# magenta/music-spectrogram-diffusion

Measured on AMD Instinct MI355X. Metric: mel-frames/sec, higher is better.
Workload: dtype f16x3 (operands split into hi + lo half planes, 3 f16 MFMAs per product, fp32 accumulate; fp32 residual/norm/softmax/sampler); 1 GPU; base_with_context, 1000-step DDPM, CFG w=5, 1 song(s) per GPU, segment-sequential with context hand-off, 5 segments of 256 frames per GPU; precision=f16x3, precision_requested=f16x3, parallelism=song-parallel x1, mode=replicas, attention_query_planes=library default: hi + lo for Q and for the softmax weights, knobs=library defaults

## Files before the change

### music-spectrogram-diffusion_amd/build_native.py

```python
from __future__ import annotations

import os
import shutil
import subprocess
import sys

HERE = os.path.dirname(os.path.abspath(__file__))
ROOT = os.path.dirname(HERE)
CSRC = os.path.join(HERE, 'csrc')
EXP = os.path.join(ROOT, 'tools', 'ubench', 'exp')
LIB = os.path.join(CSRC, 'libmsd_amd.so')
LIB_EXP = os.path.join(EXP, 'libmsd_amd_exp.so')
LIBS = {'f16': (LIB, []), 'bf16': (os.path.join(CSRC, 'libmsd_amd_bf16.so'), ['-DMSD_PLANE_BF16=1'])}
EXP_SRC = os.path.join(EXP, 'src_r04')
EXP_LIBS = {'exp': (LIB_EXP, ['-DMSD_EXPERIMENTS=1'])}
SOURCES = ['msd_api.hip']
HEADERS = ['common.h', 'phase_stamps.h', 'gemm_h16.h', 'gemm_f32.h', 'attention.h', 'elementwise.h',
           os.path.join('..', '..', 'include', 'msd_amd.h')]
EXP_HEADERS = ['chain.h', 'gemm_h16_exp.h', 'gemm_splitk_exchange.inc', 'gemm_h16_pair.h', 'gemm_h16_wide.h', 'gemm_h16_ls.h']


def _hipcc():
  for c in (os.environ.get('HIPCC'), shutil.which('hipcc'), '/opt/rocm/bin/hipcc'):
    if c and os.path.exists(c):
      return c
  raise RuntimeError('hipcc not found (ROCm toolchain required to build the HIP library)')


def needs_build(lib: str = LIB) -> bool:
  if not os.path.exists(lib):
    return True
  t = os.path.getmtime(lib)
  if os.path.abspath(lib) == os.path.abspath(LIB_EXP):
    deps = [os.path.join(EXP_SRC, f) for f in os.listdir(EXP_SRC)] + [os.path.join(EXP, f) for f in EXP_HEADERS]
  else:
    deps = [os.path.join(CSRC, f) for f in SOURCES + HEADERS + [os.path.join('..', 'build_native.py')]]
  return any(os.path.getmtime(f) > t for f in deps)


def check_prefetch_registers(listing: str) -> str:
  tool = os.path.join(HERE, 'check_prefetch_regs.py')
  if not os.path.exists(tool):
    raise RuntimeError('%s is missing: the build cannot verify the prefetch registers of the library' % tool)
  out = subprocess.run([sys.executable, tool, listing], capture_output=True, text=True)
  if out.returncode != 0:
    raise RuntimeError('prefetch register check failed on %s:\n%s\n%s' % (listing, out.stdout[-3000:], out.stderr[-2000:]))
  return out.stdout.strip().split('\n')[-1]


NO_SCRATCH_KERNELS = ('sampler_step_kernel', 'threefry_normal_kernel')


def check_no_scratch(listing: str, kernels=NO_SCRATCH_KERNELS) -> str:
  import re
  text = open(listing).read()
  seen = {k: 0 for k in kernels}
  bad = []
  for m in re.finditer(r'^\s*\.amdhsa_kernel\s+(\S+)(.*?)^\s*\.end_amdhsa_kernel', text, flags=re.M | re.S):
    name, body = m.group(1), m.group(2)
    for k in kernels:
      if k in name:
        seen[k] += 1
        size = re.search(r'\.amdhsa_private_segment_fixed_size\s+(\d+)', body)
        dyn = re.search(r'\.amdhsa_uses_dynamic_stack\s+(\d+)', body)
        if size is None or int(size.group(1)) != 0 or (dyn is not None and int(dyn.group(1)) != 0):
          bad.append('%s: private segment %s, dynamic stack %s' % (name, size.group(1) if size else '?', dyn.group(1) if dyn else '0'))
  missing = [k for k, c in seen.items() if c == 0]
  if missing:
    raise RuntimeError('scratch check: no kernel descriptor of %s in %s' % (missing, listing))
  if bad:
    raise RuntimeError('scratch check failed on %s: these kernels use scratch memory:\n  %s' % (listing, '\n  '.join(bad)))
  return 'OK: no scratch in ' + ', '.join('%d x %s' % (c, k) for k, c in seen.items())


def build(force: bool = False, verbose: bool = True, experiments: bool = False) -> str:
  import tempfile
  targets = [(lib, defs, CSRC) for lib, defs in LIBS.values()]
  if experiments:
    if not os.path.isdir(EXP_SRC):
      raise RuntimeError('%s is missing: run `bash tools/ubench/exp/restore_src_r04.sh` first (the experiments build needs round 4\'s sources)' % EXP_SRC)
    targets += [(lib, defs, EXP_SRC) for lib, defs in EXP_LIBS.values()]
  for lib, defs, src in targets:
    if not force and not needs_build(lib):
      continue
    with tempfile.TemporaryDirectory(prefix='msd_build_') as tmp:
      out = os.path.join(tmp, os.path.basename(lib))
      cmd = [_hipcc(), '--offload-arch=gfx950', '-O3', '-std=c++17', '-fPIC', '-shared', '-save-temps',
             '-fno-gpu-rdc', '-Wno-unused-result', '-ffile-prefix-map=%s=.' % ROOT, '-ffile-prefix-map=%s=.' % tmp,
             '-cuid=msd_amd',
             '-I', src] + defs + ['-o', os.path.basename(lib)] + [os.path.join(src, s) for s in SOURCES]
      if verbose:
        print('[build_native]', ' '.join(cmd), flush=True)
      subprocess.run(cmd, check=True, cwd=tmp)
      listings = [os.path.join(tmp, f) for f in os.listdir(tmp) if f.endswith('.s') and 'gfx950' in f]
      if not listings:
        raise RuntimeError('no gfx950 device listing (*gfx950*.s, -save-temps) in %s: cannot verify the prefetch '
                           'registers; the scratch directory holds %s' % (tmp, sorted(os.listdir(tmp))))
      for l in listings:
        verdict = check_prefetch_registers(l)
        if verbose:
          print('[build_native] prefetch registers:', verdict, flush=True)
        if src == CSRC:
          verdict = check_no_scratch(l)
          if verbose:
            print('[build_native] scratch:', verdict, flush=True)
      shutil.copyfile(out, lib + '.tmp')
      os.chmod(lib + '.tmp', 0o755)
      os.replace(lib + '.tmp', lib)
  return LIB


if __name__ == '__main__':
  build(force='--force' in sys.argv, experiments='--experiments' in sys.argv)
  print(LIB)
```

### music-spectrogram-diffusion_amd/csrc/gemm_h16.h

```cpp
#pragma once
#include <type_traits>
#include "common.h"
#include "phase_stamps.h"

namespace msd {

struct PrefetchTarget {
  const char* base[2] = {nullptr, nullptr};
  int rows = 0;
  int row_stride = 0;
  int lpr = 0;
  int lg = 0;
  void set(const void* p0, const void* p1, int rows_, int row_stride_, int row_bytes) {
    base[0] = static_cast<const char*>(p0); base[1] = static_cast<const char*>(p1);
    rows = rows_; row_stride = row_stride_; lpr = (row_bytes + 127) >> 7;
    lg = 0;
    while ((1 << lg) < lpr) ++lg;
  }
};
constexpr int kMaxPrefetchTargets = 1;
struct WeightPrefetch {
  PrefetchTarget t[kMaxPrefetchTargets];
  int n = 0;
  void add(const PrefetchTarget& x) { if (x.rows > 0 && n < kMaxPrefetchTargets) t[n++] = x; }
};

constexpr int kPrefetchPerThread = 3;
template <int PF>
struct PrefetchRegsT { uint32_t r[PF > 0 ? PF * kPrefetchPerThread : 1]; };
enum { kPfNone = 0 };
__host__ __device__ inline int prefetch_kind(const WeightPrefetch& pf) { return pf.n; }

template <int PF>
__device__ __forceinline__ void prefetch_weights(const WeightPrefetch& pf, int blk, int nblk, const void* valid,
                                                 PrefetchRegsT<PF>& keep) {
  if constexpr (PF == kPfNone) {
    keep.r[0] = 0;
    return;
  } else {
    const int wave = __builtin_amdgcn_readfirstlane((int)threadIdx.x >> 6), nwave = (int)blockDim.x >> 6;
    const int lane = (int)threadIdx.x & 63;
#pragma unroll
    for (int k = 0; k < PF; ++k) {
      const PrefetchTarget& t = pf.t[k];
      const int rows = t.rows, lpr = t.lpr;
      const int planes = t.base[1] && t.base[1] != t.base[0] ? 2 : 1;
      const int rpt = 64 >> t.lg;
      const int sub = lane >> t.lg, line = lane & ((1 << t.lg) - 1);
      const uint32_t lane_off = (uint32_t)sub * (uint32_t)t.row_stride + (uint32_t)line * 128u;
#pragma unroll
      for (int u = 0; u < kPrefetchPerThread; ++u) {
        const int rp0 = ((blk + nblk * u) * nwave + wave) * rpt;
        const int pl = (planes == 2 && rp0 >= rows) ? 1 : 0, row0 = rp0 - pl * rows;
        const char* row_ptr = t.base[pl] + (size_t)row0 * t.row_stride;
        const bool in = rp0 < rows * planes && row0 + sub < rows && line < lpr;
        const char* src = in ? row_ptr + lane_off : reinterpret_cast<const char*>(valid);
        asm volatile("global_load_dword %0, %1, off ; msd_prefetch" : "=&v"(keep.r[k * kPrefetchPerThread + u]) : "v"(src) : "memory");
      }
    }
  }
}
template <int PF>
__device__ __forceinline__ void prefetch_done(const PrefetchRegsT<PF>& keep) {
#pragma unroll
  for (int u = 0; u < (PF > 0 ? PF * kPrefetchPerThread : 1); ++u) asm volatile("" ::"v"(keep.r[u]));
}

constexpr bool kPfWave = true;
constexpr bool kPfWaveAttn = true;
template <int PF, bool LDS_SINK = false>
__device__ __forceinline__ void prefetch_wave(const WeightPrefetch& pf, int blk, int nblk, const void* valid,
                                              char* sink_lds = nullptr) {
  if constexpr (PF != kPfNone) {
    constexpr int TOUCHES = 4 * kPrefetchPerThread;
    const int lane = (int)threadIdx.x & 63;
    uint32_t sink = 0;
#pragma unroll
    for (int k = 0; k < PF; ++k) {
      const PrefetchTarget& t = pf.t[k];
      const int rows = t.rows, lpr = t.lpr;
      const int planes = t.base[1] && t.base[1] != t.base[0] ? 2 : 1;
      const int rpt = 64 >> t.lg;
      const int sub = lane >> t.lg, line = lane & ((1 << t.lg) - 1);
      const uint32_t lane_off = (uint32_t)sub * (uint32_t)t.row_stride + (uint32_t)line * 128u;
#pragma unroll
      for (int u = 0; u < TOUCHES; ++u) {
        const int rp0 = (blk + nblk * u) * rpt;
        const int pl = (planes == 2 && rp0 >= rows) ? 1 : 0, row0 = rp0 - pl * rows;
        const char* row_ptr = t.base[pl] + (size_t)row0 * t.row_stride;
        const bool in = rp0 < rows * planes && row0 + sub < rows && line < lpr;
        const char* src = in ? row_ptr + lane_off : reinterpret_cast<const char*>(valid);
        if constexpr (LDS_SINK) {
          typedef const __attribute__((address_space(1))) void* pf_gptr_t;
          typedef __attribute__((address_space(3))) void* pf_lptr_t;
          __builtin_amdgcn_global_load_lds((pf_gptr_t)src, (pf_lptr_t)(size_t)(unsigned)(size_t)sink_lds, 4, 0, 0);
        } else {
          asm volatile("global_load_dword %0, %1, off ; msd_prefetch" : "+v"(sink) : "v"(src) : "memory");
        }
      }
    }
    asm volatile("" ::"v"(sink));
  }
}

struct GemmParams {
  const h16_t* A[2];
  const h16_t* B[2];
  int lda, ldb;
  int M, N, K;
  WeightPrefetch pf;
  int pf_nblk = 0;
  int xcd_rows = 1;
  int xcd_walk_n = 0;
  struct TileMap {
    int nbm = 0, nbn = 0;
    int nbm_x = 1, nbn_x = 1;
    int cx_log2 = 3;
    unsigned inv_nbm_x = 0, inv_nbn_x = 0;
    void fill(int M, int N, int BM, int BN, int rx) {
      const int cx = 8 / rx;
      nbm = M / BM; nbn = N / BN;
      nbm_x = (nbm + rx - 1) / rx; nbn_x = (nbn + cx - 1) / cx;
      cx_log2 = cx == 8 ? 3 : (cx == 4 ? 2 : (cx == 2 ? 1 : 0));
      inv_nbm_x = nbm_x > 1 ? (unsigned)((0x100000000ull + (unsigned)nbm_x - 1) / (unsigned)nbm_x) : 0u;
      inv_nbn_x = nbn_x > 1 ? (unsigned)((0x100000000ull + (unsigned)nbn_x - 1) / (unsigned)nbn_x) : 0u;
    }
  } map;
  unsigned* sat = nullptr;
  unsigned sat_tag = 1;
};

struct SatFlag {
  unsigned* p = nullptr;
  unsigned tag = 1;
};

typedef __attribute__((ext_vector_type(8))) plane_elem mfma_h16x8;
typedef __attribute__((ext_vector_type(4))) unsigned int u32x4;

__device__ __forceinline__ mfma_h16x8 as_frag(uint4 v) {
  union { uint4 u; mfma_h16x8 f; } c;
  c.u = v;
  return c.f;
}

__device__ __forceinline__ mfma_h16x8 ld_frag16(const h16_t* p) {
  return as_frag(*reinterpret_cast<const uint4*>(p));
}

__device__ __forceinline__ int vt_perm16(int o) { return 8 * ((o >> 2) & 1) + (o & 3) + 4 * (o >> 3); }

constexpr int kSlabPad = 4;
constexpr int kGemmBK = 64;

__device__ __forceinline__ int lds_tile_off(int row, int chunk) {
  return row * 128 + ((chunk ^ (row & 7)) << 4);
}

template <int BM, int BN>
struct GemmAcc {
  static constexpr int FM = BM / 32, FN = BN / 32;
  f32x4 a[FM][FN];
};

template <int NP, int BM, int BN, int NS, class Epi, int PF = kPfNone, bool PROLOGUE = true, bool REG_EPI = false>
__device__ __forceinline__ void gemm_tile(const GemmParams& p, const Epi& epi, int bm, int bn, char* smem,
                                          GemmAcc<BM, BN>* acc_out = nullptr, int ts_blk = -1, bool fresh = false) {
#if MSD_TIMESTAMPS
  const int msd_ts_blk = ts_blk >= 0 ? ts_blk : (int)blockIdx.x;
#endif
  constexpr bool W13 = BN == 48;
  static_assert(!W13 || (NP == 2 && BM == 32), "1 x 3 wave layout: 32 x 48 tiles, two planes");
  constexpr int WM = W13 ? BM : BM / 2, WN = W13 ? 16 : BN / 2;
  constexpr int FM = WM / 16, FN = WN / 16;
  constexpr int A_BYTES = BM * 128, B_BYTES = BN * 128;
  constexpr int STAGE_BYTES = NP * (A_BYTES + B_BYTES);
  constexpr int A_LD = BM / 32, B_LD = BN / 32;
  constexpr int B_Q = W13 ? BN / 16 : NP * B_LD;
  constexpr int PW = NP * A_LD + B_Q;
  constexpr int LDS_LD = BN + kSlabPad;
  static_assert((BM * LDS_LD + BM) * 4 <= NS * STAGE_BYTES, "epilogue slab must fit the operand LDS");

  const int tid = threadIdx.x, lane = tid & 63;
  const int wave = __builtin_amdgcn_readfirstlane(tid >> 6);
  const int wm = W13 ? 0 : wave >> 1, wn = W13 ? (wave < 2 ? wave : 2) : wave & 1;
  const int m0 = bm * BM, n0 = bn * BN;

  const int r8 = lane >> 3, csrc = (lane & 7) ^ r8;
  const h16_t* ga[NP];
  const h16_t* gb[NP];
#pragma unroll
  for (int pl = 0; pl < NP; ++pl) {
    ga[pl] = p.A[pl] + (size_t)(m0 + wave * (BM / 4) + r8) * p.lda + csrc * 8;
    gb[pl] = W13 ? p.B[wave >> 1] + (size_t)(n0 + (wave & 1) * (BN / 2) + r8) * p.ldb + csrc * 8
                 : p.B[pl] + (size_t)(n0 + wave * (BN / 4) + r8) * p.ldb + csrc * 8;
  }
  const size_t a_step = (size_t)8 * p.lda, b_step = (size_t)8 * p.ldb;
#define MSD_A_SRC(PL, I, K0) (ga[PL] + (I) * a_step + (K0))
  typedef const __attribute__((address_space(1))) void* gptr_t;
  typedef __attribute__((address_space(3))) void* lptr_t;

#define MSD_D_ISSUE1(KT, BUF, Q)                                                             \
  {                                                                                          \
    char* base_ = smem + (BUF) * STAGE_BYTES;                                                \
    const int k0_ = (KT) * kGemmBK;                                                          \
    if constexpr (W13) {                                                                     \
      if ((Q) < NP * A_LD)                                                                   \
        __builtin_amdgcn_global_load_lds((gptr_t)(MSD_A_SRC((Q) / A_LD, (Q) % A_LD, k0_)),   \
            (lptr_t)(base_ + ((Q) / A_LD) * A_BYTES + (wave * (BM / 4) + 8 * ((Q) % A_LD)) * 128), 16, 0, 0); \
      else                                                                                   \
        __builtin_amdgcn_global_load_lds((gptr_t)(gb[0] + ((Q) - NP * A_LD) * b_step + k0_), \
            (lptr_t)(base_ + NP * A_BYTES + (wave >> 1) * B_BYTES +                          \
                     ((wave & 1) * (BN / 2) + 8 * ((Q) - NP * A_LD)) * 128), 16, 0, 0);      \
    } else {                                                                                 \
      constexpr int AB_ = A_LD + (B_LD ? B_LD : 1);                                          \
      const int     pl_ = (Q) / AB_, r_ = (Q) % AB_;                                         \
      if (r_ < A_LD)                                                                         \
        __builtin_amdgcn_global_load_lds((gptr_t)(MSD_A_SRC(pl_, r_, k0_)),                  \
            (lptr_t)(base_ + pl_ * A_BYTES + (wave * (BM / 4) + 8 * r_) * 128), 16, 0, 0);   \
      else                                                                                   \
        __builtin_amdgcn_global_load_lds((gptr_t)(gb[pl_] + (r_ - A_LD) * b_step + k0_),     \
            (lptr_t)(base_ + NP * A_BYTES + pl_ * B_BYTES + (wave * (BN / 4) + 8 * (r_ - A_LD)) * 128), 16, 0, 0); \
    }                                                                                        \
  }
#define MSD_D_ISSUE(KT, BUF)                                                                \
  { _Pragma("unroll") for (int q0_ = 0; q0_ < PW; ++q0_) MSD_D_ISSUE1(KT, BUF, q0_) }

  f32x4 acc[FM][FN];
#pragma unroll
  for (int i = 0; i < FM; ++i)
#pragma unroll
    for (int j = 0; j < FN; ++j) acc[i][j] = f32x4{0.f, 0.f, 0.f, 0.f};

  const int nk = p.K / kGemmBK;
  MSD_TS_BEGIN((ts_class<BM, BN>()), msd_ts_blk)
  if constexpr (PROLOGUE) {
#pragma unroll
    for (int s = 0; s < NS; ++s)
      if (s < nk) MSD_D_ISSUE(s, s)
  }
  char* const aux = smem + NS * STAGE_BYTES;
  if constexpr (PROLOGUE) epi.template prefetch<BM, BN>(aux, m0, n0, wave, lane);
  __builtin_amdgcn_sched_barrier(0);
  MSD_TS_STAMP(BM, BN, 1)

#define MSD_D_READ(FA, FB, BUF, KK)                                                          \
  {                                                                                          \
    const char* base_ = smem + (BUF) * STAGE_BYTES;                                          \
    const int c_ = (KK) * 4 + (lane >> 4);                                                   \
    _Pragma("unroll") for (int pl = 0; pl < NP; ++pl) {                                      \
      _Pragma("unroll") for (int i = 0; i < FM; ++i)                                         \
        FA[pl][i] = *reinterpret_cast<const mfma_h16x8*>(                                   \
            base_ + pl * A_BYTES + lds_tile_off(wm * WM + i * 16 + (lane & 15), c_));        \
      _Pragma("unroll") for (int j = 0; j < FN; ++j)                                         \
        FB[pl][j] = *reinterpret_cast<const mfma_h16x8*>(                                   \
            base_ + NP * A_BYTES + pl * B_BYTES + lds_tile_off(wn * WN + j * 16 + (lane & 15), c_)); \
    }                                                                                        \
  }

  mfma_h16x8 fa0[NP][FM], fb0[NP][FN], fa1[NP][FM], fb1[NP][FN];
  constexpr int RD = NP * (FM + FN);
  constexpr int MQ = (NP == 2 ? 3 : 1) * FM * FN;
  constexpr int SLOTS = RD > PW ? RD : PW;
  constexpr int MPR = MQ / SLOTS;
  static_assert(W13 || PW == RD, "one DMA and one fragment read per slot");
#define MSD_D_READ1(FA, FB, BUF, KK, Q)                                                      \
  {                                                                                          \
    const int     pl_ = (Q) / (FM + FN), r_ = (Q) % (FM + FN);                               \
    const char* base_ = smem + (BUF) * STAGE_BYTES;                                          \
    const int c_ = (KK) * 4 + (lane >> 4);                                                   \
    if (r_ < FM)                                                                             \
      FA[pl_][r_ < FM ? r_ : 0] = *reinterpret_cast<const mfma_h16x8*>(                     \
          base_ + pl_ * A_BYTES + lds_tile_off(wm * WM + r_ * 16 + (lane & 15), c_));        \
    else                                                                                     \
      FB[pl_][r_ < FM ? 0 : r_ - FM] = *reinterpret_cast<const mfma_h16x8*>(                \
          base_ + NP * A_BYTES + pl_ * B_BYTES + lds_tile_off(wn * WN + (r_ - FM) * 16 + (lane & 15), c_)); \
  }
#define MSD_D_MFMA1(FA, FB, E)                                                               \
  {                                                                                          \
    const int     pr_ = (E) / (FM * FN), t_ = (E) % (FM * FN), i_ = t_ / FN, j_ = t_ % FN;    \
    const int     pb_ = (pr_ == 1) ? NP - 1 : 0, pa_ = (pr_ == 2) ? NP - 1 : 0;              \
    acc[i_][j_] = MSD_MFMA_16X16X32(FB[pb_][j_], FA[pa_][i_], acc[i_][j_], 0, 0, 0); \
  }
#define MSD_D_HALF(DO_ISSUE, KT, BUF_I, FAn, FBn, BUF_R, KK, DO_READ, FAc, FBc)              \
  {                                                                                          \
    _Pragma("unroll") for (int q_ = 0; q_ < SLOTS; ++q_) {                                   \
      if (DO_ISSUE && q_ < PW) MSD_D_ISSUE1(KT, BUF_I, q_)                                   \
      if (DO_READ && q_ < RD) MSD_D_READ1(FAn, FBn, BUF_R, KK, q_)                           \
      _Pragma("unroll") for (int e_ = q_ * MPR; e_ < (q_ + 1 == SLOTS ? MQ : (q_ + 1) * MPR); ++e_) \
        MSD_D_MFMA1(FAc, FBc, e_)                                                            \
      __builtin_amdgcn_sched_barrier(0);                                                     \
    }                                                                                        \
  }
#define MSD_D_BARRIER __builtin_amdgcn_s_barrier();
#define MSD_D_DOISSUE 1
#define MSD_D_STEP(DO_ISSUE, VMWAIT)                                                         \
  {                                                                                          \
    MSD_D_HALF(0, 0, 0, fa1, fb1, buf, 1, 1, fa0, fb0)                                       \
    int nb = buf + 1;                                                                        \
    if (nb == NS) nb = 0;                                                                    \
    asm volatile("s_waitcnt vmcnt(%0)" ::"n"(VMWAIT) : "memory");      \
    __builtin_amdgcn_s_waitcnt(0xC07F);   \
    MSD_D_BARRIER                           \
    __builtin_amdgcn_sched_barrier(0);                                                       \
    MSD_D_HALF(DO_ISSUE, kt + NS, buf, fa0, fb0, nb, 0, 1, fa1, fb1)                         \
     \
     \
     \
    __builtin_amdgcn_s_waitcnt(0xC07F);                                                      \
    buf = nb;                                                                                \
  }

  if ((PROLOGUE || fresh) && nk >= NS) {
    asm volatile("s_waitcnt vmcnt(%0)" ::"n"((NS - 1) * PW) : "memory");
  } else {
    asm volatile("s_waitcnt vmcnt(0)" ::: "memory");
  }
  __builtin_amdgcn_s_barrier();
  __builtin_amdgcn_sched_barrier(0);
  MSD_TS_STAMP(BM, BN, 2)
  MSD_D_READ(fa0, fb0, 0, 0)
  __builtin_amdgcn_s_waitcnt(0xC07F);
  int buf = 0;
  int kt = 0;
  for (; kt + NS < nk; ++kt) MSD_D_STEP(MSD_D_DOISSUE, (NS - 2) * PW)
  if (nk >= NS) {
    if constexpr (NS >= 4) { if (kt + 1 < nk) { MSD_D_STEP(0, (NS - 2) * PW) ++kt; } }
    if constexpr (NS >= 3) { if (kt + 1 < nk) { MSD_D_STEP(0, (NS >= 4 ? NS - 3 : NS - 2) * PW) ++kt; } }
    if constexpr (NS >= 5) { static_assert(NS <= 4, "write the drain ladder for this ring depth"); }
  }
  for (; kt + 1 < nk; ++kt) MSD_D_STEP(0, 0)
  MSD_D_HALF(0, 0, 0, fa1, fb1, buf, 1, 1, fa0, fb0)
  MSD_D_HALF(0, 0, 0, fa0, fb0, buf, 0, 0, fa1, fb1)
#undef MSD_D_STEP
#undef MSD_D_HALF
#undef MSD_D_ISSUE1
#undef MSD_D_READ1
#undef MSD_D_MFMA1
#undef MSD_D_DOISSUE
#undef MSD_D_BARRIER
#undef MSD_D_READ
#undef MSD_D_ISSUE
#undef MSD_A_SRC
  __syncthreads();
  MSD_TS_STAMP(BM, BN, 3)
  if constexpr (REG_EPI) {
    static_assert(!W13, "register epilogues: 2 x 2 wave layout");
#pragma unroll
    for (int i = 0; i < FM; ++i)
#pragma unroll
      for (int j = 0; j < FN; ++j) acc_out->a[i][j] = acc[i][j];
    return;
  } else {
  float* slab = reinterpret_cast<float*>(smem);
  const int lm = lane & 15, ln = (lane >> 4) * 4;
  auto store_slab = [&]() {
    if (W13 && wave == 3) return;
#pragma unroll
    for (int i = 0; i < FM; ++i)
#pragma unroll
      for (int j = 0; j < FN; ++j)
        *reinterpret_cast<float4*>(slab + (size_t)(wm * WM + i * 16 + lm) * LDS_LD + wn * WN + j * 16 + ln) =
            make_float4(acc[i][j][0] * kWScaleInv, acc[i][j][1] * kWScaleInv, acc[i][j][2] * kWScaleInv,
                        acc[i][j][3] * kWScaleInv);
  };
  PrefetchRegsT<PF> pf_keep;
  if constexpr (!kPfWave) prefetch_weights<PF>(p.pf, blockIdx.x, p.pf_nblk > 0 ? p.pf_nblk : (int)gridDim.x, p.B[0], pf_keep);
  else prefetch_weights<kPfNone>(p.pf, 0, 1, nullptr, reinterpret_cast<PrefetchRegsT<kPfNone>&>(pf_keep));
  store_slab();
  epi.template stats<BM, LDS_LD>(slab, m0, tid, aux);
  __syncthreads();
  MSD_TS_STAMP(BM, BN, 4)
  epi.template run<BM, BN, LDS_LD>(slab, m0, n0, tid, aux, true, SatFlag{p.sat, p.sat_tag});
  MSD_TS_STAMP(BM, BN, 5)
  MSD_TS_END((ts_class<BM, BN>()), msd_ts_blk, gridDim.x)
  prefetch_done(pf_keep);
  }
}

__device__ __forceinline__ bool gemm_block_tile(const GemmParams& p, int b, int& bm, int& bn) {
  const GemmParams::TileMap& tm = p.map;
  const int RX = p.xcd_rows, CX = 1 << tm.cx_log2;
  const int xcd = b & 7, tt = b >> 3;
  const int xr = xcd >> tm.cx_log2, xc = xcd & (CX - 1);
  if (p.xcd_walk_n) {
    const int q = tm.nbn_x > 1 ? (int)__umulhi((unsigned)tt, tm.inv_nbn_x) : tt;
    bm = q * RX + xr; bn = (tt - q * tm.nbn_x) * CX + xc;
  } else {
    const int q = tm.nbm_x > 1 ? (int)__umulhi((unsigned)tt, tm.inv_nbm_x) : tt;
    bm = (tt - q * tm.nbm_x) * RX + xr; bn = q * CX + xc;
  }
  return bn < tm.nbn && bm < tm.nbm;
}

constexpr int pf_threads(int pf) { return kPfWave && pf != kPfNone ? 64 : 0; }

template <int NP, int BM, int BN, int NS, class Epi, int PF = kPfNone>
__global__ void __launch_bounds__(256 + pf_threads(PF)) gemm_h16_dma_kernel(GemmParams p, Epi epi) {
  extern __shared__ __attribute__((aligned(16))) char smem[];
  warm_kernargs<kernarg_lines<GemmParams, Epi>()>();
  if constexpr (kPfWave && PF != kPfNone) {
    if (threadIdx.x >= 256) {
      prefetch_wave<PF>(p.pf, blockIdx.x, gridDim.x, p.B[0]);
      return;
    }
  }
  int bm, bn;
  if (!gemm_block_tile(p, (int)blockIdx.x, bm, bn)) return;
  gemm_tile<NP, BM, BN, NS, Epi, PF>(p, epi, bm, bn, smem);
}

template <int LD>
__device__ __forceinline__ void tile_row8(const float* s0, int m, int n, float v[8]) {
  const float4 a0 = *reinterpret_cast<const float4*>(s0 + m * LD + n);
  const float4 a1 = *reinterpret_cast<const float4*>(s0 + m * LD + n + 4);
  v[0] = a0.x; v[1] = a0.y; v[2] = a0.z; v[3] = a0.w;
  v[4] = a1.x; v[5] = a1.y; v[6] = a1.z; v[7] = a1.w;
}

template <int NP>
__device__ __forceinline__ void store_h16x8(h16_t* const* planes, size_t off, const float v[8], RangeCheck& rc) {
  uint32_t wh[4], wl[4];
#pragma unroll
  for (int e = 0; e < 4; ++e) {
    rc.see(v[2 * e], v[2 * e + 1]);
    if (NP == 2) split2_h16(v[2 * e], v[2 * e + 1], wh[e], wl[e]);
    else wh[e] = cvt2_h16(v[2 * e], v[2 * e + 1]);
  }
  *reinterpret_cast<uint4*>(planes[0] + off) = make_uint4(wh[0], wh[1], wh[2], wh[3]);
  if (NP == 2) *reinterpret_cast<uint4*>(planes[1] + off) = make_uint4(wl[0], wl[1], wl[2], wl[3]);
}

struct RowScale {
  const float* ssq = nullptr;
  int tiles = 0;
  float inv_d = 0.f;
  const float* bias = nullptr;
  int bias_step_stride = 0;
  const int* step_ptr = nullptr;
};

constexpr int kAuxMaxTiles = 32;

#ifndef MSD_EPI_AUX_OPTIONAL
#define MSD_EPI_AUX_OPTIONAL 0
#endif
__device__ __forceinline__ bool aux_present(const char* aux) {
#if MSD_EPI_AUX_OPTIONAL
  return aux != nullptr;
#else
  (void)aux;
  return true;
#endif
}

typedef const __attribute__((address_space(1))) void* aux_gptr_t;
typedef __attribute__((address_space(3))) void* aux_lptr_t;

__device__ __forceinline__ aux_lptr_t lds_ptr_of(const void* generic) {
  return (aux_lptr_t)(size_t)(unsigned)(size_t)generic;
}

__device__ __forceinline__ int scan_index(const int* p) {
  int v;
  asm volatile("s_nop 4\n\ts_load_dword %0, %1, 0x0\n\ts_waitcnt lgkmcnt(0)" : "=s"(v) : "s"(p) : "memory");
  return v;
}

__device__ __forceinline__ void aux_dma_linear(const void* g, char* dst, int bytes, int wave, int lane) {
  const int n_instr = (bytes + 1023) >> 10;
  for (int i = wave; i < n_instr; i += 4) {
    int off = i * 1024 + lane * 16;
    off = off < bytes - 16 ? off : bytes - 16;
    __builtin_amdgcn_global_load_lds((aux_gptr_t)((const char*)g + off), lds_ptr_of(dst + i * 1024), 16, 0, 0);
  }
}

__device__ __forceinline__ void aux_dma_row(const void* g, char* dst, int bytes, int lane) {
  int off = lane * 16;
  off = off < bytes - 16 ? off : bytes - 16;
  __builtin_amdgcn_global_load_lds((aux_gptr_t)((const char*)g + off), lds_ptr_of(dst), 16, 0, 0);
}

template <int BM>
constexpr int rowscale_aux_bytes() { return BM * kAuxMaxTiles * 4 + 1024; }
template <int BM>
__host__ __device__ __forceinline__ int rowscale_ssq_bytes(int tiles) { return (BM * tiles * 4 + 1023) & ~1023; }

template <int BM, int BN>
__device__ __forceinline__ void rowscale_prefetch(const RowScale& r, char* aux, int m0, int n0, int wave, int lane) {
  if (!r.ssq) return;
  aux_dma_linear(r.ssq + (size_t)m0 * r.tiles, aux, BM * r.tiles * 4, wave, lane);
  if (r.bias && wave == 3)
    aux_dma_row(r.bias + (size_t)scan_index(r.step_ptr) * r.bias_step_stride + n0, aux + rowscale_ssq_bytes<BM>(r.tiles), BN * 4, lane);
}

typedef const __attribute__((address_space(3))) float* lds_cf32;

typedef const __attribute__((address_space(3))) f32x4* lds_cf32x4;
struct BiasRow {
  lds_cf32 l = nullptr;
  bool present = false;
  __device__ __forceinline__ float at(int i) const { return l[i]; }
  __device__ __forceinline__ void at8(int i, float (&b)[8]) const {
    const f32x4 b0 = reinterpret_cast<lds_cf32x4>(l + i)[0], b1 = reinterpret_cast<lds_cf32x4>(l + i)[1];
    b[0] = b0[0]; b[1] = b0[1]; b[2] = b0[2]; b[3] = b0[3];
    b[4] = b1[0]; b[5] = b1[1]; b[6] = b1[2]; b[7] = b1[3];
  }
};

template <class F>
__device__ __forceinline__ void rowscale_variants(bool folded, bool has_bias, F&& f) {
  if (!folded) f(std::integral_constant<int, 0>{});
  else if (!has_bias) f(std::integral_constant<int, 1>{});
  else f(std::integral_constant<int, 2>{});
}

template <int MODE>
__device__ __forceinline__ void rowscale8(float (&v)[8], float rs, const BiasRow& bias, int i) {
  if constexpr (MODE == 2) {
    float b[8];
    bias.at8(i, b);
#pragma unroll
    for (int e = 0; e < 8; ++e) v[e] = v[e] * rs + b[e];
  } else if constexpr (MODE == 1) {
#pragma unroll
    for (int e = 0; e < 8; ++e) v[e] = v[e] * rs + 0.f;
  }
}

#define MSD_EPI_ITEMS(ITEMS, item)                                             \
  _Pragma("unroll") for (int it_ = 0; it_ < ((ITEMS) + 255) / 256; ++it_)      \
    if (const int item = tid + it_ * 256; ((ITEMS) % 256 == 0) || item < (ITEMS))

template <int BM>
__device__ __forceinline__ void tile_rstd_compute(const RowScale& r, float* rs, int m0, int tid, const char* aux) {
  constexpr int TPR = 256 / BM;
  const int row = tid / TPR, part = tid % TPR;
  float acc = 0.f;
  if (aux_present(aux)) {
    lds_cf32 q = (lds_cf32)(aux) + row * r.tiles;
    constexpr int MAXIT = kAuxMaxTiles / TPR;
    float v[MAXIT];
#pragma unroll
    for (int i = 0; i < MAXIT; ++i) {
      const int t = part + i * TPR;
      v[i] = q[t < r.tiles ? t : part];
    }
#pragma unroll
    for (int i = 0; i < MAXIT; ++i) acc += (part + i * TPR < r.tiles) ? v[i] : 0.f;
  } else {
    const float* q = r.ssq + (size_t)(m0 + row) * r.tiles;
    for (int t = part; t < r.tiles; t += TPR) acc += q[t];
  }
#pragma unroll
  for (int o = 1; o < TPR; o <<= 1) acc += __shfl_xor(acc, o, 64);
  if (part == 0) rs[row] = 1.0f / sqrtf(acc * r.inv_d + 1e-6f);
}

template <int BM>
__device__ __forceinline__ BiasRow tile_rstd(const RowScale& r, float* rs, int m0, int n0, int tid,
                                             const char* aux, bool stats_done = false) {
  if (!stats_done) {
    tile_rstd_compute<BM>(r, rs, m0, tid, aux);
    __syncthreads();
  }
  BiasRow b;
  if (r.bias) {
    if (!aux_present(aux)) __builtin_trap();
    b.present = true;
    b.l = (lds_cf32)(aux + rowscale_ssq_bytes<BM>(r.tiles));
  }
  return b;
}

template <int NP>
struct EpiStoreH16 {
  h16_t* out[2];
  int ldc;
  RowScale rsc;
  template <int BM, int BN> static constexpr int aux_bytes() { return rowscale_aux_bytes<BM>(); }
  template <int BM, int BN>
  __device__ void prefetch(char* aux, int m0, int n0, int wave, int lane) const {
    rowscale_prefetch<BM, BN>(rsc, aux, m0, n0, wave, lane);
  }
  template <int BM, int LD>
  __device__ void stats(float* s0, int m0, int tid, const char* aux) const {
    if (rsc.ssq) tile_rstd_compute<BM>(rsc, s0 + BM * LD, m0, tid, aux);
  }
  template <int BM, int BN, int LD>
  __device__ void run(float* s0, int m0, int n0, int tid, const char* aux = nullptr, bool stats_done = false,
                      SatFlag sf = SatFlag()) const {
    float* rs = s0 + BM * LD;
    BiasRow bias;
    if (rsc.ssq) bias = tile_rstd<BM>(rsc, rs, m0, n0, tid, aux, stats_done);
    RangeCheck rc;
    rowscale_variants(rsc.ssq != nullptr, bias.present, [&](auto mode) {
      MSD_EPI_ITEMS(BM * BN / 8, item) {
        const int m = item / (BN / 8), n = (item % (BN / 8)) * 8;
        float v[8];
        tile_row8<LD>(s0, m, n, v);
        rowscale8<decltype(mode)::value>(v, decltype(mode)::value ? rs[m] : 1.f, bias, n);
        store_h16x8<NP>(out, (size_t)(m0 + m) * ldc + n0 + n, v, rc);
      }
    });
    rc.commit(sf.p, sf.tag);
  }
};

template <int NP>
struct EpiQKV {
  h16_t* qk[2];
  h16_t* vt[2];
  int ld_qk, v_start, seg_len, vt_ld, vt_rows;
  RowScale rsc;
  template <int BM, int BN> static constexpr int aux_bytes() { return rowscale_aux_bytes<BM>(); }
  template <int BM, int BN>
  __device__ void prefetch(char* aux, int m0, int n0, int wave, int lane) const {
    rowscale_prefetch<BM, BN>(rsc, aux, m0, n0, wave, lane);
  }
  template <int BM, int LD>
  __device__ void stats(float* s0, int m0, int tid, const char* aux) const {
    if (rsc.ssq) tile_rstd_compute<BM>(rsc, s0 + BM * LD, m0, tid, aux);
  }
  template <int BM, int BN, int LD>
  __device__ void run(float* s0, int m0, int n0, int tid, const char* aux = nullptr, bool stats_done = false,
                      SatFlag sf = SatFlag()) const {
    float* rs = s0 + BM * LD;
    BiasRow bias;
    if (rsc.ssq) bias = tile_rstd<BM>(rsc, rs, m0, n0, tid, aux, stats_done);
    RangeCheck rc;
    if (n0 < v_start) {
      rowscale_variants(rsc.ssq != nullptr, bias.present, [&](auto mode) {
        MSD_EPI_ITEMS(BM * BN / 8, item) {
          const int m = item / (BN / 8), n = (item % (BN / 8)) * 8;
          float v[8];
// ... 735 lines not shown
```

Measured before the change: 272.0 mel-frames/sec.

## Split LDS-DMA issue across both half steps of the GEMM main loop

```diff
diff --git a/music-spectrogram-diffusion_amd/build_native.py b/music-spectrogram-diffusion_amd/build_native.py
--- a/music-spectrogram-diffusion_amd/build_native.py
+++ b/music-spectrogram-diffusion_amd/build_native.py
@@ -1,6 +1,7 @@
 from __future__ import annotations
 
 import os
+import re
 import shutil
 import subprocess
 import sys
@@ -48,11 +49,162 @@
   return out.stdout.strip().split('\n')[-1]
 
 
+DMA_WAIT_KERNELS = ('gemm_h16_dma_kernel', 'gemm_h16_dual_kernel', 'gemm_h16_geglu_persist_kernel')
+
+
+def _dw_tile_shapes(name):
+  np_ = int(re.search(r'_kernelILi(\d+)E', name).group(1))
+  m = re.search(r'persist_kernelILi\d+ELi(\d+)ELi(\d+)ELi(\d+)E', name)
+  if m:
+    return [(np_,) + tuple(int(x) for x in m.groups())]
+  return [(np_,) + tuple(int(x) for x in t) for t in re.findall(r'Li(\d+)ELi(\d+)ELi(\d+)ENS_', name)]
+
+
+def _dw_dmas_per_wave(np_, bm, bn):
+  return np_ * (bm // 32) + (bn // 16 if bn == 48 else np_ * (bn // 32))
+
+
+def _dw_blocks_of(lines, s, end):
+  out, label, ev, loop = [], 'entry', [], False
+  for j in range(s + 1, end):
+    l = lines[j].split(';')[0].strip()
+    m = re.match(r'^(\.LBB\w+):', l)
+    if m:
+      out.append((label, ev, loop))
+      label, ev, loop = m.group(1), [], False
+    elif l.startswith('global_load_lds_dwordx4'):
+      ev.append(('D',))
+    elif l.startswith('s_waitcnt') and 'vmcnt' in l:
+      n = int(re.search(r'vmcnt\((\d+)\)', l).group(1))
+      ev.append(('W' if 'msd_tile_wait' in lines[j] else 'w', n))
+    elif l.startswith('s_barrier'):
+      ev.append(('B',))
+    elif l.startswith('v_mfma'):
+      ev.append(('M',))
+    elif l.startswith(('s_cbranch', 's_branch')) and l.split()[-1] == label:
+      loop = True
+  out.append((label, ev, loop))
+  return out
+
+
+def _dw_replay(ns, pw, entry, steady, drain, nk, aux):
+  issued, last_op = 0, {}
+  for t in range(min(nk, ns)):
+    issued += pw
+    last_op[t] = issued
+  issued += aux
+  def wait(n, need, what):
+    if issued - n < last_op[need]:
+      return '%s: vmcnt(%d) with %d operations issued leaves tile %d (complete at operation %d) in flight' % (what, n, issued, need, last_op[need])
+    return None
+  bad = wait(entry if nk >= ns else 0, 0, 'entry, nk = %d' % nk)
+  kt = 0
+  while bad is None and kt + ns < nk:
+    bad = wait(steady, kt + 1, 'steady state, nk = %d, step %d' % (nk, kt))
+    if bad is None and aux == 0 and issued - steady != last_op[kt + 1]:
+      bad = 'steady state: vmcnt(%d) drains younger tiles than the one it needs (%d operations issued, tile %d ends at %d)' % (steady, issued, kt + 1, last_op[kt + 1])
+    issued += pw
+    last_op[kt + ns] = issued
+    kt += 1
+  ladder = list(drain) if nk >= ns else []
+  while bad is None and kt + 1 < nk:
+    n = ladder.pop(0) if ladder else 0
+    bad = wait(n, kt + 1, 'drain, nk = %d, step %d' % (nk, kt))
+    kt += 1
+  return bad
+
+
+def _dw_check_kernel(name, blocks):
+  shapes = _dw_tile_shapes(name)
+  if not shapes:
+    return ['cannot read the tile shape from the name']
+  errs = []
+  loops = [(lab, ev) for lab, ev, loop in blocks if loop and any(e[0] == 'D' for e in ev) and any(e[0] == 'W' for e in ev)]
+  tile_waits = [(lab, ev) for lab, ev, loop in blocks if any(e[0] == 'W' for e in ev)]
+  want = sorted((_dw_dmas_per_wave(np_, bm, bn), ns) for np_, bm, bn, ns in shapes)
+  if len(loops) != len(shapes):
+    return ['%d steady-state loops for %d tile bodies' % (len(loops), len(shapes))]
+  found = []
+  for lab, ev in loops:
+    kinds = [e[0] for e in ev]
+    nd = kinds.count('D')
+    if kinds.count('W') != 1 or kinds.count('B') != 1 or 'w' in kinds:
+      errs.append('%s: a steady-state loop holds exactly one tile wait, one barrier and no other vmcnt wait: %s' % (lab, [e for e in ev if e[0] in 'WwB']))
+      continue
+    if not kinds.index('W') < kinds.index('B') < kinds.index('D'):
+      errs.append('%s: the loop issues LDS-DMAs in front of its tile wait and barrier (the slot they refill is not free yet)' % lab)
+    found.append((nd, next(e[1] for e in ev if e[0] == 'W')))
+  by_pw = {}
+  for nd, n in found:
+    by_pw.setdefault(nd, set()).add(n)
+  for pw, ns in want:
+    if pw not in by_pw:
+      errs.append('no steady-state loop issues PW = %d DMAs (found %s)' % (pw, sorted(by_pw)))
+    elif by_pw[pw] != {(ns - 2) * pw}:
+      errs.append('PW = %d, NS = %d: steady-state wait vmcnt%s, expected (NS - 2) PW = %d' % (pw, ns, sorted(by_pw[pw]), (ns - 2) * pw))
+  if errs:
+    return errs
+  entry, drain = set(), []
+  loop_labels = {lab for lab, _ in loops}
+  for lab, ev in tile_waits:
+    if lab in loop_labels:
+      continue
+    kinds = [e[0] for e in ev]
+    if 'D' in kinds[kinds.index('W'):]:
+      errs.append('%s: LDS-DMA behind a tile wait outside the steady-state loop' % lab)
+    n = next(e[1] for e in ev if e[0] == 'W')
+    if 'M' in kinds[kinds.index('W'):]:
+      drain.append(n)
+    else:
+      entry.add(n)
+  for pw, ns in set(want):
+    ladder = [n for n in ((ns - 2) * pw, (ns - 3) * pw) if n > 0]
+    full = (ns - 1) * pw
+    if full not in entry or 0 not in entry:
+      errs.append('PW = %d, NS = %d: entry waits %s, expected vmcnt(%d) and vmcnt(0)' % (pw, ns, sorted(entry), full))
+    for n in ladder:
+      if n not in drain:
+        errs.append('PW = %d, NS = %d: no drain step waits with vmcnt(%d) (drain steps: %s)' % (pw, ns, n, sorted(drain)))
+    if 0 not in drain:
+      errs.append('PW = %d, NS = %d: no drain step waits with vmcnt(0)' % (pw, ns))
+    for nk in range(1, ns + 5):
+      for aux in (0, 3):
+        bad = _dw_replay(ns, pw, full, (ns - 2) * pw, ladder, nk, aux)
+        if bad:
+          errs.append('PW = %d, NS = %d: %s' % (pw, ns, bad))
+  allowed = {n for pw, ns in want for n in ((ns - 2) * pw, (ns - 3) * pw, 0) if n >= 0}
+  for n in drain:
+    if n not in allowed:
+      errs.append('a drain step waits with vmcnt(%d), which no tile shape of this kernel explains (%s)' % (n, sorted(allowed)))
+  allowed_entry = {0} | {(ns - 1) * pw for pw, ns in want}
+  for n in entry:
+    if n not in allowed_entry:
+      errs.append('an entry wait is vmcnt(%d), which no tile shape of this kernel explains (%s)' % (n, sorted(allowed_entry)))
+  return errs
+
+
+def check_dma_waits(listing: str) -> str:
+  lines = open(listing).read().split('\n')
+  starts = [i for i, l in enumerate(lines) if re.match(r'^_Z\w+:', l)]
+  n, bad = 0, []
+  for k, s in enumerate(starts):
+    name = lines[s].split(':')[0]
+    if not any(kn in name for kn in DMA_WAIT_KERNELS):
+      continue
+    end = starts[k + 1] if k + 1 < len(starts) else len(lines)
+    n += 1
+    bad += ['%s: %s' % (name[:120], e) for e in _dw_check_kernel(name, _dw_blocks_of(lines, s, end))]
+  if n == 0:
+    raise RuntimeError('DMA wait check: no GEMM kernel in %s' % listing)
+  if bad:
+    raise RuntimeError('DMA wait check failed on %s:\n  %s' % (listing, '\n  '.join(bad[:40])))
+  return 'OK: %d GEMM kernels, counted waits consistent' % n
+
+
 NO_SCRATCH_KERNELS = ('sampler_step_kernel', 'threefry_normal_kernel')
 
 
 def check_no_scratch(listing: str, kernels=NO_SCRATCH_KERNELS) -> str:
-  import re
   text = open(listing).read()
   seen = {k: 0 for k in kernels}
   bad = []
@@ -104,6 +256,9 @@
           verdict = check_no_scratch(l)
           if verbose:
             print('[build_native] scratch:', verdict, flush=True)
+          verdict = check_dma_waits(l)
+          if verbose:
+            print('[build_native] counted DMA waits:', verdict, flush=True)
       shutil.copyfile(out, lib + '.tmp')
       os.chmod(lib + '.tmp', 0o755)
       os.replace(lib + '.tmp', lib)
diff --git a/music-spectrogram-diffusion_amd/csrc/gemm_h16.h b/music-spectrogram-diffusion_amd/csrc/gemm_h16.h
--- a/music-spectrogram-diffusion_amd/csrc/gemm_h16.h
+++ b/music-spectrogram-diffusion_amd/csrc/gemm_h16.h
@@ -282,10 +282,14 @@
     const int     pb_ = (pr_ == 1) ? NP - 1 : 0, pa_ = (pr_ == 2) ? NP - 1 : 0;              \
     acc[i_][j_] = MSD_MFMA_16X16X32(FB[pb_][j_], FA[pa_][i_], acc[i_][j_], 0, 0, 0); \
   }
-#define MSD_D_HALF(DO_ISSUE, KT, BUF_I, FAn, FBn, BUF_R, KK, DO_READ, FAc, FBc)              \
+  constexpr bool SPLIT = NS >= 3;
+  constexpr int H1 = SPLIT ? (PW + 1) / 2 : PW;
+  constexpr int QS = SPLIT ? 2 : 1;
+  static_assert((H1 - 1) * QS < SLOTS, "the DMAs of a half step fit its slots");
+#define MSD_D_HALF(DO_ISSUE, KT, BUF_I, Q0, QN, FAn, FBn, BUF_R, KK, DO_READ, FAc, FBc)      \
   {                                                                                          \
     _Pragma("unroll") for (int q_ = 0; q_ < SLOTS; ++q_) {                                   \
-      if (DO_ISSUE && q_ < PW) MSD_D_ISSUE1(KT, BUF_I, q_)                                   \
+      if (DO_ISSUE && q_ % QS == 0 && q_ / QS < (QN)) MSD_D_ISSUE1(KT, BUF_I, (Q0) + q_ / QS) \
       if (DO_READ && q_ < RD) MSD_D_READ1(FAn, FBn, BUF_R, KK, q_)                           \
       _Pragma("unroll") for (int e_ = q_ * MPR; e_ < (q_ + 1 == SLOTS ? MQ : (q_ + 1) * MPR); ++e_) \
         MSD_D_MFMA1(FAc, FBc, e_)                                                            \
@@ -296,25 +300,25 @@
 #define MSD_D_DOISSUE 1
 #define MSD_D_STEP(DO_ISSUE, VMWAIT)                                                         \
   {                                                                                          \
-    MSD_D_HALF(0, 0, 0, fa1, fb1, buf, 1, 1, fa0, fb0)                                       \
     int nb = buf + 1;                                                                        \
     if (nb == NS) nb = 0;                                                                    \
-    asm volatile("s_waitcnt vmcnt(%0)" ::"n"(VMWAIT) : "memory");      \
+    asm volatile("s_waitcnt vmcnt(%0) ; msd_tile_wait" ::"n"(VMWAIT) : "memory");  \
     __builtin_amdgcn_s_waitcnt(0xC07F);   \
     MSD_D_BARRIER                           \
     __builtin_amdgcn_sched_barrier(0);                                                       \
-    MSD_D_HALF(DO_ISSUE, kt + NS, buf, fa0, fb0, nb, 0, 1, fa1, fb1)                         \
+    MSD_D_HALF(DO_ISSUE, kt + NS, buf, 0, H1, fa0, fb0, nb, 0, 1, fa1, fb1)                  \
      \
      \
      \
     __builtin_amdgcn_s_waitcnt(0xC07F);                                                      \
+    MSD_D_HALF(DO_ISSUE && SPLIT, kt + NS, buf, H1, PW - H1, fa1, fb1, nb, 1, 1, fa0, fb0)   \
     buf = nb;                                                                                \
   }
 
   if ((PROLOGUE || fresh) && nk >= NS) {
-    asm volatile("s_waitcnt vmcnt(%0)" ::"n"((NS - 1) * PW) : "memory");
+    asm volatile("s_waitcnt vmcnt(%0) ; msd_tile_wait" ::"n"((NS - 1) * PW) : "memory");
   } else {
-    asm volatile("s_waitcnt vmcnt(0)" ::: "memory");
+    asm volatile("s_waitcnt vmcnt(0) ; msd_tile_wait" ::: "memory");
   }
   __builtin_amdgcn_s_barrier();
   __builtin_amdgcn_sched_barrier(0);
@@ -323,6 +327,7 @@
   __builtin_amdgcn_s_waitcnt(0xC07F);
   int buf = 0;
   int kt = 0;
+  MSD_D_HALF(0, 0, 0, 0, 0, fa1, fb1, buf, 1, 1, fa0, fb0)
   for (; kt + NS < nk; ++kt) MSD_D_STEP(MSD_D_DOISSUE, (NS - 2) * PW)
   if (nk >= NS) {
     if constexpr (NS >= 4) { if (kt + 1 < nk) { MSD_D_STEP(0, (NS - 2) * PW) ++kt; } }
@@ -330,8 +335,7 @@
     if constexpr (NS >= 5) { static_assert(NS <= 4, "write the drain ladder for this ring depth"); }
   }
   for (; kt + 1 < nk; ++kt) MSD_D_STEP(0, 0)
-  MSD_D_HALF(0, 0, 0, fa1, fb1, buf, 1, 1, fa0, fb0)
-  MSD_D_HALF(0, 0, 0, fa0, fb0, buf, 0, 0, fa1, fb1)
+  MSD_D_HALF(0, 0, 0, 0, 0, fa0, fb0, buf, 0, 0, fa1, fb1)
 #undef MSD_D_STEP
 #undef MSD_D_HALF
 #undef MSD_D_ISSUE1
```

Result: no change. 273.2 mel-frames/sec (median of 6 runs) (+0.5%).
